# shivangchopra11/MedMoE

Measured on AMD Instinct MI355X. Metric: image-text pairs/sec at global batch 1024, higher is better.
Workload: dtype bf16; 1 GPU; cfg2: ViT-B/16 + 12-layer text tower (frozen), 8 experts top-2, 224x224x3 + 77 tokens, fwd+bwd+clip+Adam; global_batch=1024, per_gpu_batch=1024, parallelism=dp1

## Files before the change

medmoe_amd/csrc/pair3.hip:

```cpp
#include "common.h"

struct Pair3Args {
  const uint16_t* lp; bf16_t* dS; bf16_t* A; bf16_t* U;
  const float* lse; const bf16_t* gm; const float* wnorm; float* stats; float* d2; float* dwn;
  const int* cap_lens; const float* gsim; float* sim; float* att; const int* cap_list;
  long long row_base, ld, bstride;
  int n_cap, B, Bc, HW, HWP, T, caps_per_wg, n_chunk, pw;
  long long stat_rows;
  float temp1, temp2, eps;
};

template <int CTRL>
__device__ __forceinline__ float dpp_mov(float v) {
  return __builtin_bit_cast(float, __builtin_amdgcn_update_dpp(0, __builtin_bit_cast(int, v), CTRL, 0xf, 0xf, true));
}
__device__ __forceinline__ float row16_sum(float v) {
  v += dpp_mov<0xB1>(v);
  v += dpp_mov<0x4E>(v);
  v += dpp_mov<0x141>(v);
  v += dpp_mov<0x140>(v);
  return v;
}
#define P3_DPP4(CTRL)                                                                                          \
  "v_add_f32_dpp %0, %0, %0 " CTRL " row_mask:0xf bank_mask:0xf\n\tv_add_f32_dpp %1, %1, %1 " CTRL " row_mask:0xf bank_mask:0xf\n\t" \
  "v_add_f32_dpp %2, %2, %2 " CTRL " row_mask:0xf bank_mask:0xf\n\tv_add_f32_dpp %3, %3, %3 " CTRL " row_mask:0xf bank_mask:0xf\n\t"
__device__ __forceinline__ void row16_sum4(float& a, float& b, float& c, float& d) {
  asm volatile("s_nop 1\n\t" P3_DPP4("quad_perm:[1,0,3,2]") P3_DPP4("quad_perm:[2,3,0,1]") P3_DPP4("row_half_mirror") P3_DPP4("row_mirror")
               : "+v"(a), "+v"(b), "+v"(c), "+v"(d));
}
__device__ __forceinline__ float grp4_sum(float v) {
  v += __shfl_xor(v, 16, 64);
  v += __shfl_xor(v, 32, 64);
  return v;
}
__device__ __forceinline__ uint32_t dword_of(const uint4& v, int d) { return d == 0 ? v.x : d == 1 ? v.y : d == 2 ? v.z : v.w; }
__device__ __forceinline__ void opaque(uint4& v) { asm volatile("" : "+v"(v.x), "+v"(v.y), "+v"(v.z), "+v"(v.w)); }
__device__ __forceinline__ float bf_lo(uint32_t w) { return __uint_as_float(w << 16); }
__device__ __forceinline__ float bf_hi(uint32_t w) { return __uint_as_float(w & 0xffff0000u); }
__device__ __forceinline__ void lds_store_b32(unsigned addr, unsigned v) { asm volatile("ds_write_b32 %0, %1" :: "v"(addr), "v"(v) : "memory"); }
__device__ __forceinline__ unsigned lds_load_b32(unsigned addr) {
  unsigned v;
  asm volatile("ds_read_b32 %0, %1\n\ts_waitcnt lgkmcnt(0)" : "=v"(v) : "v"(addr) : "memory");
  return v;
}
__device__ __forceinline__ void flag_publish(unsigned addr, int epoch) {
  asm volatile("s_waitcnt lgkmcnt(0)" ::: "memory");
  lds_store_b32(addr, (unsigned)epoch);
}
__device__ __forceinline__ void flag_wait(unsigned addr, int epoch) {
  while ((int)__builtin_amdgcn_readfirstlane(lds_load_b32(addr)) < epoch) __builtin_amdgcn_s_sleep(1);
}

template <int HW, int NTT, bool BWD, bool WN = false>
__global__ __launch_bounds__(1024) void local_pair3_kernel(Pair3Args p) {
  constexpr int NS = (HW + 31) / 32, HWP = ((HW + 15) / 16) * 16;
  const int pw = p.pw;
  constexpr int NRT = 2 * NS, GR = NS * 32, CPI = 16 / NTT, TP = NTT * 16;
  constexpr int NRTA = (HW - 32 * (NS - 1) > 4) ? NRT : NRT - 1;
  constexpr int OFF_L = NRT * NS * 1024, OFF_R = OFF_L + 16 * GR * 4, OFF_E = OFF_R + 2 * 16 * GR * 4, OFF_F = OFF_E + 128;
  __shared__ __attribute__((aligned(16))) char smem[OFF_F + 128];
  const int tid = threadIdx.x, lane = tid & 63, wid = __builtin_amdgcn_readfirstlane(tid >> 6);
  const int fr = lane & 15, g = lane >> 4;
  const int pid = blockIdx.x;
  const int b = pid / p.n_chunk, chunk = pid - b * p.n_chunk;
  float* Lw = (float*)(smem + OFF_L) + wid * GR;
  float* Rbase = (float*)(smem + OFF_R);
  const unsigned lds0 = (unsigned)(size_t)smem;
  const unsigned eboxA = lds0 + OFF_E, flagE = lds0 + OFF_F, flagR = flagE + 64;
  if (tid < 32) ((int*)(smem + OFF_F))[tid] = 0;
  for (int f = wid; f < NRT * NS; f += 16) {
    const int rt = f / NS, s = f - rt * NS;
    const int row = 32 * (rt >> 1) + 8 * (fr >> 2) + 4 * (rt & 1) + (fr & 3);
    *(uint4*)(smem + f * 1024 + lane * 16) = *(const uint4*)(p.gm + ((long long)b * GR + row) * GR + 32 * s + 8 * g);
  }
  __syncthreads();
  const int grp = wid / NTT, tt = wid - grp * NTT, w0 = grp * NTT;
  if (grp >= CPI) return;
  const float c1 = p.temp1 * 1.44269504088896f;
  constexpr float LN2 = 0.6931471805599453f;
  const int j_end = min(p.n_cap, (chunk + 1) * p.caps_per_wg);
  constexpr uint32_t hmin = 0xFB53u;
  const char* gfrag = smem + lane * 16;
  auto load_frags = [&](bf16x8_t (&f)[NS], int rt) __attribute__((always_inline)) {
#pragma unroll
    for (int s = 0; s < NS; ++s) f[s] = *(const bf16x8_t*)(gfrag + (rt * NS + s) * 1024);
  };
  int epoch = 0;
  for (int j = chunk * p.caps_per_wg + grp; j < j_end; j += CPI) {
    ++epoch;
    const int i = p.cap_list ? p.cap_list[j] : j;
    const int cap = max(1, min(min(p.cap_lens[i], p.T), TP));
    const int t = tt * 16 + fr;
    const float mcol = t < cap ? 1.f : 0.f;
    const float nw = p.wnorm[i * p.T + min(t, p.T - 1)];
    const float gs = (BWD && p.gsim) ? p.gsim[(long long)b * p.Bc + i] : 1.f;
    const float simv = BWD ? p.sim[(long long)b * p.Bc + i] : 0.f;
    float2 st = make_float2(0.f, 0.f);
    if (BWD) st = *(const float2*)(p.stats + ((long long)b * p.stat_rows + p.row_base + (long long)j * TP + tt * 16 + fr) * 2);
    const long long off0 = (p.row_base + (long long)j * TP + t) * p.ld + (long long)b * p.bstride + 8 * g;
    uint4 lpv[NS];
#pragma unroll
    for (int s = 0; s < NS; ++s) {
      const int h0 = 32 * s + 8 * g;
      if (32 * s + 31 < HW) lpv[s] = *(const uint4*)(p.lp + off0 + 32 * s);
      else lpv[s] = (h0 < pw) ? *(const uint4*)(p.lp + off0 + 32 * s) : make_uint4(LOGP_MIN_BITS2, LOGP_MIN_BITS2, LOGP_MIN_BITS2, LOGP_MIN_BITS2);
      if (32 * s + 31 >= HW) {
        auto fix = [&](uint32_t w, int d) -> uint32_t {
          if (h0 + 2 * d >= HW) w = (w & 0xffff0000u) | hmin;
          if (h0 + 2 * d + 1 >= HW) w = (w & 0x0000ffffu) | (hmin << 16);
          return w;
        };
        lpv[s] = make_uint4(fix(lpv[s].x, 0), fix(lpv[s].y, 1), fix(lpv[s].z, 2), fix(lpv[s].w, 3));
      }
    }
    if (lane * 4 < GR) {
      const int h0 = lane * 4;
      float4 v = make_float4(0.f, 0.f, 0.f, 0.f);
      if (h0 < HWP) v = *(const float4*)(p.lse + ((long long)b * p.Bc + i) * HWP + h0);
      if (h0 >= HW) v.x = 0.f;
      if (h0 + 1 >= HW) v.y = 0.f;
      if (h0 + 2 >= HW) v.z = 0.f;
      if (h0 + 3 >= HW) v.w = 0.f;
      *(float4*)(Lw + h0) = v;
    }
    auto lp_of = [&](int s, int e) -> float {
      const uint32_t w = dword_of(lpv[s], e >> 1);
      return h2f((uint16_t)((e & 1) ? (w >> 16) : (w & 0xffffu)));
    };
    uint4 af[NS];
    float num, n2;
    if constexpr (BWD) {
#pragma unroll
      for (int s = 0; s < NS; ++s) af[s] = (32 * s + 31 < HW || 32 * s + 8 * g < pw) ? *(const uint4*)(p.A + off0 + 32 * s) : make_uint4(0u, 0u, 0u, 0u);
    }
    auto a_of = [&](int s, int e) -> float {
      const uint32_t w = dword_of(af[s], e >> 1);
      return (e & 1) ? bf_hi(w) : bf_lo(w);
    };
    bf16x8_t fg[NS];
    auto y_tile = [&](int next) __attribute__((always_inline)) -> f32x4_t {
      f32x4_t y = {0.f, 0.f, 0.f, 0.f};
#pragma unroll
      for (int s = 0; s < NS; ++s) y = __builtin_amdgcn_mfma_f32_16x16x32_bf16(fg[s], __builtin_bit_cast(bf16x8_t, af[s]), y, 0, 0, 0);
      __builtin_amdgcn_sched_barrier(0);
      if (next >= 0) load_frags(fg, next);
      __builtin_amdgcn_sched_barrier(0);
      return y;
    };
    auto y_tile_now = [&](int rt) __attribute__((always_inline)) -> f32x4_t {
      bf16x8_t f[NS];
      load_frags(f, rt);
      f32x4_t y = {0.f, 0.f, 0.f, 0.f};
#pragma unroll
      for (int s = 0; s < NS; ++s) y = __builtin_amdgcn_mfma_f32_16x16x32_bf16(f[s], __builtin_bit_cast(bf16x8_t, af[s]), y, 0, 0, 0);
      __builtin_amdgcn_sched_barrier(0);
      return y;
    };
    if constexpr (!BWD) {
      float e1[NS][8];
      float cs = 0.f, un = 0.f;
  #pragma unroll
      for (int s = 0; s < NS; ++s) {
        const float4 La = *(const float4*)(Lw + 32 * s + 8 * g), Lb = *(const float4*)(Lw + 32 * s + 8 * g + 4);
        const float Ls[8] = {La.x, La.y, La.z, La.w, Lb.x, Lb.y, Lb.z, Lb.w};
  #pragma unroll
        for (int e = 0; e < 8; ++e) {
          const float lp = lp_of(s, e);
          const float a1 = __builtin_amdgcn_exp2f(lp);
          float x = __builtin_amdgcn_exp2f(c1 * a1);
          if (32 * s + 24 + e >= HW) x = (32 * s + 8 * g + e < HW) ? x : 0.f;
          e1[s][e] = x;
          cs += x;
          un += x * fmaf(lp, LN2, Ls[e]);
        }
        __builtin_amdgcn_sched_barrier(0);
      }
      cs = grp4_sum(cs);
      un = grp4_sum(un);
      const float cinv = mcol / fmaxf(cs, 1e-30f);
      num = un * cinv;
  #pragma unroll
      for (int s = 0; s < NS; ++s) {
        float a[8];
  #pragma unroll
        for (int e = 0; e < 8; ++e) a[e] = e1[s][e] * cinv;
        const uint4 av = make_uint4(pack2bf(a[0], a[1]), pack2bf(a[2], a[3]), pack2bf(a[4], a[5]), pack2bf(a[6], a[7]));
        af[s] = av;
        if (32 * s + 31 < HW || 32 * s + 8 * g < pw) *(uint4*)(p.A + off0 + 32 * s) = av;
      }
      __builtin_amdgcn_sched_barrier(0);
  #pragma unroll
      for (int s = 0; s < NS; ++s) { opaque(lpv[s]); opaque(af[s]); }
      load_frags(fg, 0);
      n2 = 0.f;
  #pragma unroll
      for (int rt = 0; rt < NRTA; ++rt) {
        const f32x4_t y = y_tile(rt + 1 < NRTA ? rt + 1 : -1);
  #pragma unroll
        for (int r = 0; r < 4; ++r) n2 += a_of(rt >> 1, 4 * (rt & 1) + r) * y[r];
        __builtin_amdgcn_sched_barrier(0);
      }
      n2 = grp4_sum(n2);
      if (g == 0) *(float2*)(p.stats + ((long long)b * p.stat_rows + p.row_base + (long long)j * TP + t) * 2) = make_float2(num, n2);
    } else {
      num = st.x; n2 = st.y;
    }
    const float n2c = fmaxf(n2, 0.f);
    const float den = nw * sqrtf(n2c);
    const float cosv = num / fmaxf(den, p.eps);
    const float ev = (t < cap) ? __expf(p.temp2 * cosv) : 0.f;
    float se;
    if constexpr (!BWD) {
      se = row16_sum(ev);
      if (NTT > 1) {
        const unsigned eb = eboxA + (epoch & 1) * 64;
        lds_store_b32(eb + wid * 4, __float_as_uint(se));
        flag_publish(flagE + wid * 4, epoch);
        se = 0.f;
#pragma unroll
        for (int q = 0; q < NTT; ++q) {
          flag_wait(flagE + (w0 + q) * 4, epoch);
          se += __uint_as_float(lds_load_b32(eb + (w0 + q) * 4));
        }
      }
    } else se = __expf(simv);
    if (!BWD) {
      if (tt == 0 && lane == 0) p.sim[(long long)b * p.Bc + i] = __logf(se);
      if (p.att && b == i && t < p.T) {
#pragma unroll
        for (int s = 0; s < NS; ++s)
#pragma unroll
          for (int e = 0; e < 8; ++e) {
            const int hw = 32 * s + 8 * g + e;
            if (hw < HW) p.att[((long long)i * p.T + t) * HW + hw] = a_of(s, e);
          }
      }
      continue;
    }
    float dn = 0.f, d2 = 0.f;
    {
      const float dcos = gs * p.temp2 * ev / se;
      if (den >= p.eps) { dn = dcos / den; d2 = -dcos * cosv / fmaxf(n2c, 1e-30f); }
      else dn = dcos / p.eps;
      if (WN && g == 0)
        p.dwn[(long long)b * p.stat_rows + p.row_base + (long long)j * TP + t] = (den >= p.eps) ? -dcos * cosv / (nw * nw) : 0.f;
    }
    const float ca = dn * num + d2 * n2;
    const float k1 = p.temp1 * dn, k2 = p.temp1 * d2, k3 = p.temp1 * ca;
#pragma unroll
    for (int s = 0; s < NS; ++s) { opaque(lpv[s]); opaque(af[s]); }
    if (p.d2 && g == 0) p.d2[(long long)b * p.stat_rows + p.row_base + (long long)j * TP + t] = d2;

    if (p.U) {
#pragma unroll
      for (int s = 0; s < NS; ++s) {
        if (32 * s + 31 < HW || 32 * s + 8 * g < pw) {
          float u[8];
#pragma unroll
          for (int e = 0; e < 8; ++e) u[e] = a_of(s, e) * d2;
          *(uint4*)(p.U + off0 + 32 * s) = make_uint4(pack2bf(u[0], u[1]), pack2bf(u[2], u[3]), pack2bf(u[4], u[5]), pack2bf(u[6], u[7]));
        }
      }
    }
    __builtin_amdgcn_sched_barrier(0);
    float* Rall = Rbase + (epoch & 1) * 16 * GR;
    float* Rw = Rall + wid * GR;
#pragma unroll
    for (int s = 0; s < NS; ++s) { opaque(lpv[s]); opaque(af[s]); }
#pragma unroll
    for (int rt = 0; rt < NRTA; ++rt) {
      const int sp = rt >> 1, h = rt & 1;
      const float4 L4 = *(const float4*)(Lw + 32 * sp + 8 * g + 4 * h);
      const f32x4_t y = y_tile_now(rt);
      const float Lr[4] = {L4.x, L4.y, L4.z, L4.w};
      float pr[4];
#pragma unroll
      for (int r = 0; r < 4; ++r) {
        const float lp = lp_of(sp, 4 * h + r);
        const float a1 = __builtin_amdgcn_exp2f(lp);
        const float a = a_of(sp, 4 * h + r);
        pr[r] = a1 * (a * (k1 * fmaf(lp, LN2, Lr[r]) + (k2 * y[r] - k3)));
      }
      row16_sum4(pr[0], pr[1], pr[2], pr[3]);
      if (fr == 0) *(float4*)(Rw + 32 * sp + 8 * g + 4 * h) = make_float4(pr[0], pr[1], pr[2], pr[3]);
      __builtin_amdgcn_sched_barrier(0);
    }
    if (NTT > 1) {
      flag_publish(flagR + wid * 4, epoch);
#pragma unroll
      for (int q = 0; q < NTT; ++q) flag_wait(flagR + (w0 + q) * 4, epoch);
    }
#pragma unroll
    for (int s = 0; s < NS; ++s) { opaque(lpv[s]); opaque(af[s]); }
#pragma unroll
    for (int sp = 0; sp < NS; ++sp) {
      float ds[8];
#pragma unroll
      for (int h = 0; h < 2; ++h) {
        const int rt = 2 * sp + h;
        if (rt < NRTA) {
          const float4 L4 = *(const float4*)(Lw + 32 * sp + 8 * g + 4 * h);
          float rd[4] = {0.f, 0.f, 0.f, 0.f};
#pragma unroll
          for (int q = 0; q < NTT; ++q) {
            const float4 v = *(const float4*)(Rall + (w0 + q) * GR + 32 * sp + 8 * g + 4 * h);
            rd[0] += v.x; rd[1] += v.y; rd[2] += v.z; rd[3] += v.w;
          }
          const f32x4_t y = y_tile_now(rt);
          const float Lr[4] = {L4.x, L4.y, L4.z, L4.w};
#pragma unroll
          for (int r = 0; r < 4; ++r) {
            const float lp = lp_of(sp, 4 * h + r);
            const float a1 = __builtin_amdgcn_exp2f(lp);
            const float a = a_of(sp, 4 * h + r);
            const float da1 = a * (k1 * fmaf(lp, LN2, Lr[r]) + (k2 * y[r] - k3));
            ds[4 * h + r] = dn * a + a1 * (da1 - rd[r]);
          }
        } else {
#pragma unroll
          for (int r = 0; r < 4; ++r) ds[4 * h + r] = 0.f;
        }
        __builtin_amdgcn_sched_barrier(0);
      }
      if (32 * sp + 31 < HW || 32 * sp + 8 * g < pw)
        *(uint4*)(p.dS + off0 + 32 * sp) = make_uint4(pack2bf(ds[0], ds[1]), pack2bf(ds[2], ds[3]), pack2bf(ds[4], ds[5]), pack2bf(ds[6], ds[7]));
    }
  }
}

static int g_pair3_chunks = 0;
extern "C" int medmoe_local_pair3_chunks(int n) {
  if (n < 0) return MM_ERR_ARG;
  g_pair3_chunks = n;
  return MM_OK;
}

extern "C" int medmoe_local_pair3_supported(int HW, int T) {
  const int ntt = (T + 15) / 16;
  return ((HW == 64 && ntt == 1) || (HW == 196 && ntt >= 1 && ntt <= 5)) ? 1 : 0;
}

static int pair3_launch(const void* lp, void* dS, void* A, void* U, const float* lse, const void* gm, const float* wnorm,
                        const int* cap_lens, const float* gsim, float* sim, float* att, float* stats, long long stat_rows,
                        int B, int Bc, int HW, int T, float temp1, float temp2, float eps, const int* cap_list, int n_cap,
                        int ntt, long long row_base, long long ld, long long bstride, int pw, float* d2, float* dwn, hipStream_t stream);

extern "C" int medmoe_local_pair3(const void* lp, void* dS, void* A, void* U, const float* lse, const void* gm, const float* wnorm,
                                  const int* cap_lens, const float* gsim, float* sim, float* att, float* stats, long long stat_rows,
                                  int B, int Bc, int HW, int T, float temp1, float temp2, float eps, const int* cap_list, int n_cap,
                                  int ntt, long long row_base, long long ld, long long bstride, int pw, float* d2, hipStream_t stream) {
  return pair3_launch(lp, dS, A, U, lse, gm, wnorm, cap_lens, gsim, sim, att, stats, stat_rows, B, Bc, HW, T, temp1, temp2, eps, cap_list, n_cap, ntt,
                      row_base, ld, bstride, pw, d2, nullptr, stream);
}

extern "C" int medmoe_local_pair3_wgrad(const void* lp, void* dS, void* A, void* U, const float* lse, const void* gm, const float* wnorm,
                                        const int* cap_lens, const float* gsim, float* sim, float* att, float* stats, long long stat_rows,
                                        int B, int Bc, int HW, int T, float temp1, float temp2, float eps, const int* cap_list, int n_cap,
                                        int ntt, long long row_base, long long ld, long long bstride, int pw, float* d2, float* dwn,
                                        hipStream_t stream) {
  if (!dS || !dwn) return MM_ERR_ARG;
  return pair3_launch(lp, dS, A, U, lse, gm, wnorm, cap_lens, gsim, sim, att, stats, stat_rows, B, Bc, HW, T, temp1, temp2, eps, cap_list, n_cap, ntt,
                      row_base, ld, bstride, pw, d2, dwn, stream);
}

static int pair3_launch(const void* lp, void* dS, void* A, void* U, const float* lse, const void* gm, const float* wnorm,
                        const int* cap_lens, const float* gsim, float* sim, float* att, float* stats, long long stat_rows,
                        int B, int Bc, int HW, int T, float temp1, float temp2, float eps, const int* cap_list, int n_cap,
                        int ntt, long long row_base, long long ld, long long bstride, int pw, float* d2, float* dwn, hipStream_t stream) {
  if (dS && !U && !d2) return MM_ERR_ARG;
  if (!lp || !lse || !gm || !wnorm || !cap_lens || !A || !sim || !stats) return MM_ERR_ARG;
  if (stat_rows < row_base + (long long)n_cap * ntt * 16) return MM_ERR_SHAPE;
  if (B <= 0 || Bc <= 0 || n_cap <= 0 || (ld % 8) || (bstride % 8) || (pw % 8) || pw < HW || pw > ((HW + 31) / 32) * 32 || ntt < 1 || ntt > 5 || ntt * 16 > ((T + 15) / 16) * 16) return MM_ERR_SHAPE;
  if (!medmoe_local_pair3_supported(HW, ntt * 16)) return MM_ERR_SHAPE;
  Pair3Args p;
  p.lp = (const uint16_t*)lp; p.dS = (bf16_t*)dS; p.A = (bf16_t*)A; p.U = (bf16_t*)U;
  p.lse = lse; p.gm = (const bf16_t*)gm; p.wnorm = wnorm; p.stats = stats; p.d2 = d2; p.dwn = dwn; p.stat_rows = stat_rows; p.cap_lens = cap_lens; p.gsim = gsim; p.sim = sim; p.att = att;
  p.cap_list = cap_list; p.row_base = row_base; p.ld = ld; p.bstride = bstride; p.n_cap = n_cap; p.B = B; p.Bc = Bc; p.HW = HW;
  p.HWP = ((HW + 15) / 16) * 16; p.pw = pw; p.T = T; p.temp1 = temp1; p.temp2 = temp2; p.eps = eps;
  const int cpi = 16 / ntt;
  int n_chunk = g_pair3_chunks > 0 ? g_pair3_chunks : max(1, (1024 + B - 1) / B);
  int cpw = ((n_cap + n_chunk - 1) / n_chunk + cpi - 1) / cpi * cpi;
  n_chunk = (n_cap + cpw - 1) / cpw;
  p.caps_per_wg = cpw; p.n_chunk = n_chunk;
  const dim3 grid(B * n_chunk), block(1024);
#define P3(HW_, T_)                                                                                       \
  { if (dS && dwn) hipLaunchKernelGGL((local_pair3_kernel<HW_, T_, true, true>), grid, block, 0, stream, p);   \
    else if (dS) hipLaunchKernelGGL((local_pair3_kernel<HW_, T_, true>), grid, block, 0, stream, p);           \
    else hipLaunchKernelGGL((local_pair3_kernel<HW_, T_, false>), grid, block, 0, stream, p); }
  if (HW == 64) P3(64, 1)
  else switch (ntt) { case 1: P3(196, 1) break; case 2: P3(196, 2) break; case 3: P3(196, 3) break; case 4: P3(196, 4) break; default: P3(196, 5) break; }
#undef P3
  return mm_check_launch();
}
```

Measured before the change: 4777 pairs/s.

## Pipeline cross-wave row reduction per slab with per-slab flags in pair3 backward

Replaces the single full barrier between computing per-wave row partials and computing dS with per-slab epoch flags. Each slab's partial is published, then the previous slab's dS is finished while the next is computed, so waits overlap with compute. The da1 value is computed once and carried instead of being recomputed. A ballot-based group wait replaces the sequential per-wave flag polls. For NTT==1 the row sum is used directly with no LDS round trip. This adds register pressure from the carried values and makes the flag protocol more complex, since flag values now encode epoch*8+slab.

```diff
diff --git a/medmoe_amd/csrc/pair3.hip b/medmoe_amd/csrc/pair3.hip
--- a/medmoe_amd/csrc/pair3.hip
+++ b/medmoe_amd/csrc/pair3.hip
@@ -49,6 +49,12 @@
 }
 __device__ __forceinline__ void flag_wait(unsigned addr, int epoch) {
   while ((int)__builtin_amdgcn_readfirstlane(lds_load_b32(addr)) < epoch) __builtin_amdgcn_s_sleep(1);
+}
+
+template <int N>
+__device__ __forceinline__ void flag_wait_group(unsigned addr0, int lane, int value) {
+  const unsigned addr = addr0 + min(lane, N - 1) * 4;
+  while (__builtin_amdgcn_ballot_w64((int)lds_load_b32(addr) < value) != 0) __builtin_amdgcn_s_sleep(1);
 }
 
 template <int HW, int NTT, bool BWD, bool WN = false>
@@ -265,65 +271,85 @@
     __builtin_amdgcn_sched_barrier(0);
     float* Rall = Rbase + (epoch & 1) * 16 * GR;
     float* Rw = Rall + wid * GR;
+    const int fl0 = epoch * 8 + 1;
+    auto finish_block = [&](int sp, const float (&da)[8]) __attribute__((always_inline)) {
+      flag_wait_group<NTT>(flagR + w0 * 4, lane, fl0 + sp);
+      float ds[8];
+#pragma unroll
+      for (int h = 0; h < 2; ++h) {
+        if (2 * sp + h < NRTA) {
+          float rd[4] = {0.f, 0.f, 0.f, 0.f};
+#pragma unroll
+          for (int q = 0; q < NTT; ++q) {
+            const float4 v = *(const float4*)(Rall + (w0 + q) * GR + 32 * sp + 8 * g + 4 * h);
+            rd[0] += v.x; rd[1] += v.y; rd[2] += v.z; rd[3] += v.w;
+          }
+#pragma unroll
+          for (int r = 0; r < 4; ++r) {
+            const float a1 = __builtin_amdgcn_exp2f(lp_of(sp, 4 * h + r));
+            const float a = a_of(sp, 4 * h + r);
+            ds[4 * h + r] = dn * a + a1 * (da[4 * h + r] - rd[r]);
+          }
+        } else {
+#pragma unroll
+          for (int r = 0; r < 4; ++r) ds[4 * h + r] = 0.f;
+        }
+        __builtin_amdgcn_sched_barrier(0);
+      }
+      if (32 * sp + 31 < HW || 32 * sp + 8 * g < pw)
+        *(uint4*)(p.dS + off0 + 32 * sp) = make_uint4(pack2bf(ds[0], ds[1]), pack2bf(ds[2], ds[3]), pack2bf(ds[4], ds[5]), pack2bf(ds[6], ds[7]));
+      __builtin_amdgcn_sched_barrier(0);
+    };
 #pragma unroll
     for (int s = 0; s < NS; ++s) { opaque(lpv[s]); opaque(af[s]); }
-#pragma unroll
-    for (int rt = 0; rt < NRTA; ++rt) {
-      const int sp = rt >> 1, h = rt & 1;
-      const float4 L4 = *(const float4*)(Lw + 32 * sp + 8 * g + 4 * h);
-      const f32x4_t y = y_tile_now(rt);
-      const float Lr[4] = {L4.x, L4.y, L4.z, L4.w};
-      float pr[4];
-#pragma unroll
-      for (int r = 0; r < 4; ++r) {
-        const float lp = lp_of(sp, 4 * h + r);
-        const float a1 = __builtin_amdgcn_exp2f(lp);
-        const float a = a_of(sp, 4 * h + r);
-        pr[r] = a1 * (a * (k1 * fmaf(lp, LN2, Lr[r]) + (k2 * y[r] - k3)));
-      }
-      row16_sum4(pr[0], pr[1], pr[2], pr[3]);
-      if (fr == 0) *(float4*)(Rw + 32 * sp + 8 * g + 4 * h) = make_float4(pr[0], pr[1], pr[2], pr[3]);
-      __builtin_amdgcn_sched_barrier(0);
-    }
-    if (NTT > 1) {
-      flag_publish(flagR + wid * 4, epoch);
-#pragma unroll
-      for (int q = 0; q < NTT; ++q) flag_wait(flagR + (w0 + q) * 4, epoch);
-    }
-#pragma unroll
-    for (int s = 0; s < NS; ++s) { opaque(lpv[s]); opaque(af[s]); }
+    float dap[8];
 #pragma unroll
     for (int sp = 0; sp < NS; ++sp) {
-      float ds[8];
+      float dac[8], ds[8];
 #pragma unroll
       for (int h = 0; h < 2; ++h) {
         const int rt = 2 * sp + h;
         if (rt < NRTA) {
           const float4 L4 = *(const float4*)(Lw + 32 * sp + 8 * g + 4 * h);
-          float rd[4] = {0.f, 0.f, 0.f, 0.f};
-#pragma unroll
-          for (int q = 0; q < NTT; ++q) {
-            const float4 v = *(const float4*)(Rall + (w0 + q) * GR + 32 * sp + 8 * g + 4 * h);
-            rd[0] += v.x; rd[1] += v.y; rd[2] += v.z; rd[3] += v.w;
-          }
           const f32x4_t y = y_tile_now(rt);
           const float Lr[4] = {L4.x, L4.y, L4.z, L4.w};
+          float pr[4], a1[4];
 #pragma unroll
           for (int r = 0; r < 4; ++r) {
             const float lp = lp_of(sp, 4 * h + r);
-            const float a1 = __builtin_amdgcn_exp2f(lp);
+            a1[r] = __builtin_amdgcn_exp2f(lp);
             const float a = a_of(sp, 4 * h + r);
             const float da1 = a * (k1 * fmaf(lp, LN2, Lr[r]) + (k2 * y[r] - k3));
-            ds[4 * h + r] = dn * a + a1 * (da1 - rd[r]);
+            dac[4 * h + r] = da1;
+            pr[r] = a1[r] * da1;
+          }
+          row16_sum4(pr[0], pr[1], pr[2], pr[3]);
+          if (NTT > 1) {
+            if (fr == 0) *(float4*)(Rw + 32 * sp + 8 * g + 4 * h) = make_float4(pr[0], pr[1], pr[2], pr[3]);
+          } else {
+#pragma unroll
+            for (int r = 0; r < 4; ++r) ds[4 * h + r] = dn * a_of(sp, 4 * h + r) + a1[r] * (dac[4 * h + r] - pr[r]);
           }
         } else {
 #pragma unroll
-          for (int r = 0; r < 4; ++r) ds[4 * h + r] = 0.f;
+          for (int r = 0; r < 4; ++r) { dac[4 * h + r] = 0.f; ds[4 * h + r] = 0.f; }
         }
         __builtin_amdgcn_sched_barrier(0);
       }
-      if (32 * sp + 31 < HW || 32 * sp + 8 * g < pw)
+      if (NTT > 1) {
+        flag_publish(flagR + wid * 4, fl0 + sp);
+        if (sp > 0) {
+          opaque(lpv[sp - 1]); opaque(af[sp - 1]);
+          finish_block(sp - 1, dap);
+        }
+#pragma unroll
+        for (int e = 0; e < 8; ++e) dap[e] = dac[e];
+      } else if (32 * sp + 31 < HW || 32 * sp + 8 * g < pw)
         *(uint4*)(p.dS + off0 + 32 * sp) = make_uint4(pack2bf(ds[0], ds[1]), pack2bf(ds[2], ds[3]), pack2bf(ds[4], ds[5]), pack2bf(ds[6], ds[7]));
+    }
+    if (NTT > 1) {
+      opaque(lpv[NS - 1]); opaque(af[NS - 1]);
+      finish_block(NS - 1, dap);
     }
   }
 }
```

Result: faster. 4834 pairs/s (median of 6 runs) (+1.2%).
